# D-Hank/NeRF-tiny

Measured on AMD Instinct MI355X. Metric: rays/sec (64 coarse + 128 fine samples), lego 400x400, higher is better.
Workload: dtype f32

## Files before the change

### nerf-tiny_amd/csrc/field_bwd_reg.hip

```cpp
#include "field_common.h"

namespace nerf {

constexpr int RMB = 32;

template <int NFT>
struct WStageB {
  float4 w[NFT];
};

__device__ __forceinline__ float f4cb(const float4& v, int c) { return c == 0 ? v.x : (c == 1 ? v.y : (c == 2 ? v.z : v.w)); }

__device__ __forceinline__ unsigned mask_word(const uint16_t* __restrict__ mlayer, int t) { return mlayer[((t & 1) * 2) * 256 + (t >> 1) * 64]; }

template <int KB, int NFT, int NKB, int NNFT, bool ZERO_INIT, bool MASK_IN, bool STORE = true, bool HAS_NEXT_MASK = MASK_IN>
__device__ __forceinline__ void reg_layer_bwd(const int seg, const int next_seg , int lane,
                                              const f32x16* prev, f32x16* acc, WStageB<8>& st0, const uint16_t* __restrict__ mlayer,
                                              const uint16_t* __restrict__ mnext, unsigned& mfirst, float* __restrict__ grow, const RegBuf& rb) {
  constexpr int KT = KB / 4;
  WStageB<8> st1;
  const f32x16 zero = {0.f, 0.f, 0.f, 0.f, 0.f, 0.f, 0.f, 0.f, 0.f, 0.f, 0.f, 0.f, 0.f, 0.f, 0.f, 0.f};
  f32x16 tin[2];
  unsigned mw = mfirst;
  auto activate = [&](int t) {
    unsigned mn = 0;
    if (MASK_IN) {
      if (t + 1 < KT) mn = mask_word(mlayer, t + 1);
      else if (mnext != nullptr) mfirst = mask_word(mnext, 0);
    }
#pragma unroll
    for (int r = 0; r < 16; ++r) tin[t & 1][r] = MASK_IN ? (((mw >> r) & 1u) ? prev[t][r] : 0.f) : prev[t][r];
    if (grow == nullptr) {
#pragma unroll
      for (int r = 0; r < 16; ++r) asm volatile("" : "+v"(tin[t & 1][r]));
    }
    if (grow != nullptr) {
#pragma unroll
      for (int g = 0; g < 4; ++g)
        store_row4(grow + 32 * t + 8 * g, make_float4(tin[t & 1][4 * g], tin[t & 1][4 * g + 1], tin[t & 1][4 * g + 2], tin[t & 1][4 * g + 3]));
    }
    if (MASK_IN) mw = mn;
  };
  activate(0);
  auto kblock = [&](int kb, const WStageB<8>& cur, WStageB<8>& ld) {
    if (kb + 1 < KB) {
#pragma unroll
      for (int f = 0; f < NFT; ++f) ld.w[f] = reg_ldw(rb, seg + (int)(f * KB + kb + 1) * 64);
    } else if (next_seg >= 0) {
#pragma unroll
      for (int f = 0; f < NNFT; ++f) ld.w[f] = reg_ldw(rb, next_seg + (int)(f * NKB) * 64);
    }
    __builtin_amdgcn_sched_barrier(0);
    if ((kb & 3) == 2 && (kb >> 2) + 1 < KT) activate((kb >> 2) + 1);
#pragma unroll
    for (int s = 0; s < 4; ++s) {
      const float b = tin[(kb >> 2) & 1][4 * (kb & 3) + s];
#pragma unroll
      for (int f = 0; f < NFT; ++f) {
        if (ZERO_INIT && kb == 0 && s == 0)
          acc[f] = __builtin_amdgcn_mfma_f32_32x32x2f32(f4cb(cur.w[f], s), b, zero, 0, 0, 0);
        else
          acc[f] = __builtin_amdgcn_mfma_f32_32x32x2f32(f4cb(cur.w[f], s), b, acc[f], 0, 0, 0);
      }
    }
  };
#pragma unroll
  for (int kb = 0; kb < KB; kb += 2) {
    kblock(kb, st0, st1);
    kblock(kb + 1, st1, st0);
  }
}

template <int KB, int NKB, int NNFT, bool ZERO_INIT, bool STORE, bool HAS_NEXT_MASK>
__device__ __forceinline__ void reg_layer_bwd_thin(const int seg, const int next_seg , int lane,
                                                   const f32x16* prev, f32x16* acc, WStageB<8>& st0, const uint16_t* __restrict__ mlayer,
                                                   const uint16_t* __restrict__ mnext, unsigned& mfirst, float* __restrict__ grow, const RegBuf& rb) {
  static_assert(KB == 32, "ring indexing below assumes 32 k-blocks");
  constexpr int KT = KB / 4, D = 8;
  WStageB<8> st1;
  const f32x16 zero = {0.f, 0.f, 0.f, 0.f, 0.f, 0.f, 0.f, 0.f, 0.f, 0.f, 0.f, 0.f, 0.f, 0.f, 0.f, 0.f};
  f32x16 tin[2];
  unsigned mw = mfirst;
  auto slot = [&](int kb, int f) -> float4& { return ((kb % D) < 4) ? st0.w[2 * (kb % 4) + f] : st1.w[2 * (kb % 4) + f]; };
  auto activate = [&](int t) {
    unsigned mn = 0;
    if (t + 1 < KT) mn = mask_word(mlayer, t + 1);
    else if (HAS_NEXT_MASK) mfirst = mask_word(mnext, 0);
#pragma unroll
    for (int r = 0; r < 16; ++r) tin[t & 1][r] = ((mw >> r) & 1u) ? prev[t][r] : 0.f;
    if (STORE) {
#pragma unroll
      for (int g = 0; g < 4; ++g)
        store_row4(grow + 32 * t + 8 * g, make_float4(tin[t & 1][4 * g], tin[t & 1][4 * g + 1], tin[t & 1][4 * g + 2], tin[t & 1][4 * g + 3]));
    } else {
#pragma unroll
      for (int r = 0; r < 16; ++r) asm volatile("" : "+v"(tin[t & 1][r]));
    }
    mw = mn;
  };
#pragma unroll
  for (int kb = 1; kb < D; ++kb)
#pragma unroll
    for (int f = 0; f < 2; ++f) slot(kb, f) = reg_ldw(rb, seg + (int)(f * KB + kb) * 64);
  activate(0);
#pragma unroll
  for (int kb = 0; kb < KB; ++kb) {
    if ((kb & 3) == 2 && (kb >> 2) + 1 < KT) activate((kb >> 2) + 1);
    const float4 w0 = slot(kb, 0), w1 = slot(kb, 1);
#pragma unroll
    for (int s = 0; s < 4; ++s) {
      const float b = tin[(kb >> 2) & 1][4 * (kb & 3) + s];
      if (ZERO_INIT && kb == 0 && s == 0) {
        acc[0] = __builtin_amdgcn_mfma_f32_32x32x2f32(f4cb(w0, s), b, zero, 0, 0, 0);
        acc[1] = __builtin_amdgcn_mfma_f32_32x32x2f32(f4cb(w1, s), b, zero, 0, 0, 0);
      } else {
        acc[0] = __builtin_amdgcn_mfma_f32_32x32x2f32(f4cb(w0, s), b, acc[0], 0, 0, 0);
        acc[1] = __builtin_amdgcn_mfma_f32_32x32x2f32(f4cb(w1, s), b, acc[1], 0, 0, 0);
      }
    }
    __builtin_amdgcn_sched_barrier(0);
    if (kb + D < KB) {
#pragma unroll
      for (int f = 0; f < 2; ++f) slot(kb, f) = reg_ldw(rb, seg + (int)(f * KB + kb + D) * 64);
    } else if (kb == KB - 4 && next_seg >= 0) {
#pragma unroll
      for (int f = 0; f < NNFT; ++f) st0.w[f] = reg_ldw(rb, next_seg + (int)(f * NKB) * 64);
    }
    __builtin_amdgcn_sched_barrier(0);
  }
}

#ifdef NERF_STAMPS
#define BSTAMP(slot)                                            \
  do {                                                          \
    __builtin_amdgcn_sched_barrier(0);                          \
    const unsigned long long t_ = __builtin_readcyclecounter(); \
    __builtin_amdgcn_sched_barrier(0);                          \
    tsum[slot] += t_ - tlast;                                   \
    tlast = t_;                                                 \
  } while (0)
#else
#define BSTAMP(slot) do { } while (0)
#endif

template <bool FINE, bool QUERY = false, bool RGB = true>
__global__ __launch_bounds__(64, 1) void k_field_bwd_reg(const FieldBwdArgs a) {
  static_assert(FINE || !QUERY, "the query form carries the chain back to the points");
#ifdef NERF_STAMPS
  unsigned long long tsum[8] = {0, 0, 0, 0, 0, 0, 0, 0};
  unsigned long long tlast = __builtin_readcyclecounter();
#endif
  const int lane = threadIdx.x, j = lane & 31, h = lane >> 5;
  const int m0 = blockIdx.x * RMB;
  const int m = m0 + j;
  const bool valid = m < a.M;
  const int mc = valid ? m : a.M - 1;
  const size_t MS = (size_t)a.MSrows * WIDTH;
  const long long rrow = valid ? (long long)(a.row0 + m) : a.Mtot + j;
  const size_t grow_off = (size_t)rrow * WIDTH + 4 * h;
  float* const grow = a.G + grow_off;
  const float* const srow = a.save + grow_off;
  const uint16_t* const mrow = a.masks + ((size_t)(a.tile0 + (m0 >> 6)) * 4 + ((m0 >> 5) & 1)) * 256 + h * 32 + j;
  const size_t MKS = (size_t)a.tiles_tot * 4 * 256;
  const RegBuf rb = reg_buf(a.wp, threadIdx.x);
  constexpr int L256 = 8 * 32 * 64;
  const f32x16 zero = {0.f, 0.f, 0.f, 0.f, 0.f, 0.f, 0.f, 0.f, 0.f, 0.f, 0.f, 0.f, 0.f, 0.f, 0.f, 0.f};

  WStageB<8> st0;
  if constexpr (RGB) {
#pragma unroll
    for (int f = 0; f < 8; ++f) st0.w[f] = reg_ldw(rb, seg_off4(SEG_T_FOLD) + (f * 16) * 64);
  } else {
#pragma unroll
    for (int f = 0; f < 8; ++f) st0.w[f] = reg_ldw(rb, seg_off4(SEG_T_L7) + (f * 32) * 64);
  }
  auto mlayer = [&](int layer) { return mrow + (size_t)layer * MKS; };
  unsigned mfirst = mask_word(mlayer(7), 0);

  f32x16 D0[4];
  float ds;
  {
    const float* crow = QUERY ? a.save + (size_t)a.MSrows * QGRAD_GP + (size_t)rrow * QGRAD_C + 4 * h : srow + S_C * MS;
    float4 cv[4][4];
    float dz[3];
    if constexpr (RGB) {
#pragma unroll
      for (int t = 0; t < 4; ++t)
#pragma unroll
        for (int g = 0; g < 4; ++g) cv[t][g] = *reinterpret_cast<const float4*>(crow + 32 * t + 8 * g);
#pragma unroll
      for (int ch = 0; ch < 3; ++ch) {
        const float o = a.rgb[(size_t)mc * 3 + ch];
        const float up = a.drgb[(size_t)mc * 3 + ch];
        dz[ch] = valid ? up * ((1.0f - o) * o) : 0.f;
      }
    }
    const float sp = a.spre[a.row0 + mc];
    const float sgn = sp > 0.f ? 1.0f : (sp < 0.f ? -1.0f : 0.f);
    if constexpr (QUERY)
      ds = valid ? (a.dsig != nullptr ? a.dsig[mc] : 1.0f) * sgn : 0.f;
    else
      ds = valid ? a.dsig[mc] * sgn : 0.f;
    if (!QUERY && valid && h == 0) {
      *reinterpret_cast<float4*>(a.dz + (size_t)(a.row0 + m) * 4) = make_float4(dz[0], dz[1], dz[2], ds);
      a.dspre[a.row0 + m] = ds;
    }
    const float* wc = a.w.p[W_COLOR] + 4 * h;
#pragma unroll
    for (int t = 0; t < (RGB ? 4 : 0); ++t) {
      float4 q0[4], q1[4], q2[4];
#pragma unroll
      for (int g = 0; g < 4; ++g) {
        q0[g] = *reinterpret_cast<const float4*>(wc + 32 * t + 8 * g);
        q1[g] = *reinterpret_cast<const float4*>(wc + HALF + 32 * t + 8 * g);
        q2[g] = *reinterpret_cast<const float4*>(wc + 2 * HALF + 32 * t + 8 * g);
      }
      __builtin_amdgcn_sched_barrier(0);
#pragma unroll
      for (int g = 0; g < 4; ++g) {
        const float v0 = __builtin_fmaf(q2[g].x, dz[2], __builtin_fmaf(q1[g].x, dz[1], q0[g].x * dz[0]));
        const float v1 = __builtin_fmaf(q2[g].y, dz[2], __builtin_fmaf(q1[g].y, dz[1], q0[g].y * dz[0]));
        const float v2 = __builtin_fmaf(q2[g].z, dz[2], __builtin_fmaf(q1[g].z, dz[1], q0[g].z * dz[0]));
        const float v3 = __builtin_fmaf(q2[g].w, dz[2], __builtin_fmaf(q1[g].w, dz[1], q0[g].w * dz[0]));
        D0[t][4 * g + 0] = cv[t][g].x > 0.f ? v0 : 0.f;
        D0[t][4 * g + 1] = cv[t][g].y > 0.f ? v1 : 0.f;
        D0[t][4 * g + 2] = cv[t][g].z > 0.f ? v2 : 0.f;
        D0[t][4 * g + 3] = cv[t][g].w > 0.f ? v3 : 0.f;
      }
      __builtin_amdgcn_sched_barrier(0);
    }
  }
  BSTAMP(0);
  f32x16 A[8], B[8];
  {
    const float dsb = (h == 0) ? ds : 0.f;
    const float* ws = a.w.p[W_SIGMA];
#pragma unroll
    for (int f = 0; f < 8; ++f) B[f] = __builtin_amdgcn_mfma_f32_32x32x2f32(ws[f * 32 + j], dsb, zero, 0, 0, 0);
  }
  if constexpr (RGB)
    reg_layer_bwd<16, 8, 32, 8, false, false>(seg_off4(SEG_T_FOLD), seg_off4(SEG_T_L7), lane, D0, B, st0, nullptr, nullptr, mfirst,
                                              QUERY ? a.G : grow + G_D * MS, rb);
  BSTAMP(1);
  BSTAMP(2);
  constexpr int sT7 = seg_off4(SEG_T_L7);
  reg_layer_bwd<32, 8, 32, 8, true, true>(sT7, sT7 + L256, lane, B, A, st0, mlayer(7), mlayer(6), mfirst, QUERY ? a.G : grow + 7 * MS, rb);
  reg_layer_bwd<32, 8, 32, 8, true, true>(sT7 + L256, sT7 + 2 * L256, lane, A, B, st0, mlayer(6), mlayer(5), mfirst, QUERY ? a.G : grow + 6 * MS, rb);
  reg_layer_bwd<32, 8, 32, 8, true, true>(sT7 + 2 * L256, seg_off4(SEG_T_L4A), lane, B, A, st0, mlayer(5), mlayer(4), mfirst, QUERY ? a.G : grow + 5 * MS, rb);
  BSTAMP(3);
  f32x16 accg[2];
  if (FINE) {
    reg_layer_bwd<32, 8, 32, 2, true, true>(seg_off4(SEG_T_L4A), seg_off4(SEG_T_L4B), lane, A, B, st0, mlayer(4), mlayer(4), mfirst, QUERY ? a.G : grow + 4 * MS, rb);
    reg_layer_bwd_thin<32, 32, 8, true, false, true>(seg_off4(SEG_T_L4B), seg_off4(SEG_T_L3), lane, A, accg, st0, mlayer(4), mlayer(3), mfirst, nullptr, rb);
  } else {
    reg_layer_bwd<32, 8, 32, 8, true, true>(seg_off4(SEG_T_L4A), seg_off4(SEG_T_L3), lane, A, B, st0, mlayer(4), mlayer(3), mfirst, grow + 4 * MS, rb);
  }
  BSTAMP(4);
  constexpr int sT3 = seg_off4(SEG_T_L3);
  reg_layer_bwd<32, 8, 32, 8, true, true>(sT3, sT3 + L256, lane, B, A, st0, mlayer(3), mlayer(2), mfirst, QUERY ? a.G : grow + 3 * MS, rb);
  reg_layer_bwd<32, 8, 32, 8, true, true>(sT3 + L256, sT3 + 2 * L256, lane, A, B, st0, mlayer(2), mlayer(1), mfirst, QUERY ? a.G : grow + 2 * MS, rb);
  unsigned mb0[8];
  if (!FINE) {
#pragma unroll
    for (int t = 0; t < 8; ++t) mb0[t] = mask_word(mlayer(0), t);
  }
  reg_layer_bwd<32, 8, 32, 2, true, true, true, FINE>(sT3 + 2 * L256, FINE ? seg_off4(SEG_T_L0) : -1, lane, B, A, st0, mlayer(1),
                                                      mlayer(0), mfirst, QUERY ? a.G : grow + 1 * MS, rb);
  BSTAMP(5);
  if (FINE) {
    reg_layer_bwd_thin<32, 32, 2, false, !QUERY, false>(seg_off4(SEG_T_L0), -1, lane, A, accg, st0, mlayer(0), nullptr, mfirst,
                                                        QUERY ? nullptr : grow, rb);
    const int lane_e = __builtin_amdgcn_mbcnt_hi(~0u, __builtin_amdgcn_mbcnt_lo(~0u, 0u));
    const int j_e = lane_e & 31, h_e = lane_e >> 5;
    const int m_e = blockIdx.x * RMB + j_e;
    const bool valid_e = m_e < a.M;
    const int mc_e = valid_e ? m_e : a.M - 1;
    const long long rrow_e = valid_e ? (long long)(a.row0 + m_e) : a.Mtot + j_e;
    const float* rf = QUERY ? nullptr : a.rayf + (size_t)(mc_e / a.N) * RAYF;
    const float* gprow = QUERY ? a.save + (size_t)rrow_e * QGRAD_GP + 4 * h_e : a.save + (size_t)rrow_e * WIDTH + 4 * h_e + S_GP * ((size_t)a.MSrows * WIDTH);
    float4 gq[8];
#pragma unroll
    for (int g8 = 0; g8 < 8; ++g8) gq[g8] = *reinterpret_cast<const float4*>(gprow + 8 * g8);
    float dp[3] = {0.f, 0.f, 0.f};
#pragma unroll
    for (int g8 = 0; g8 < 8; ++g8)
#pragma unroll
      for (int e = 0; e < 2; ++e) {
        const int pi = 4 * g8 + 2 * h_e + e;
        if (pi < 30) {
          const int c = pi / 10, l = pi - 10 * c;
          const float fl = __uint_as_float(kFreqPointBits[l]);
          const float sn = e == 0 ? gq[g8].x : gq[g8].z, cn = e == 0 ? gq[g8].y : gq[g8].w;
          const float dgs = accg[g8 >> 2][4 * (g8 & 3) + 2 * e], dgc = accg[g8 >> 2][4 * (g8 & 3) + 2 * e + 1];
          const float contrib = fl * (cn * dgs - sn * dgc);
          if (c == 0) dp[0] += contrib; else if (c == 1) dp[1] += contrib; else dp[2] += contrib;
        }
      }
#pragma unroll
    for (int c = 0; c < 3; ++c) dp[c] += __shfl_xor(dp[c], 32);
    if (QUERY && valid_e && h_e == 0) {
#pragma unroll
      for (int c = 0; c < 3; ++c) a.dt[(size_t)m_e * 3 + c] = dp[c];
    }
    if (!QUERY && valid_e && h_e == 0) {
      const float dtp = __builtin_fmaf(rf[RF_DWRD + 2], dp[2], __builtin_fmaf(rf[RF_DWRD + 1], dp[1], rf[RF_DWRD] * dp[0]));
      a.dt[m_e] += dtp;
    }
  } else {
#pragma unroll
    for (int t = 0; t < 8; ++t)
#pragma unroll
      for (int g = 0; g < 4; ++g) {
        float4 v;
        v.x = ((mb0[t] >> (4 * g + 0)) & 1u) ? A[t][4 * g + 0] : 0.f;
        v.y = ((mb0[t] >> (4 * g + 1)) & 1u) ? A[t][4 * g + 1] : 0.f;
        v.z = ((mb0[t] >> (4 * g + 2)) & 1u) ? A[t][4 * g + 2] : 0.f;
        v.w = ((mb0[t] >> (4 * g + 3)) & 1u) ? A[t][4 * g + 3] : 0.f;
        store_row4(grow + 32 * t + 8 * g, v);
      }
  }
#ifdef NERF_STAMPS
  BSTAMP(6);
  if (a.stamps && lane == 0) {
    for (int i = 0; i < 7; ++i) atomicAdd(a.stamps + (FINE ? 8 : 0) + i, tsum[i]);
    atomicAdd(a.stamps + (FINE ? 30 : 31), 1ull);
  }
#endif
}

hipError_t launch_query_grad_bwd(const FieldBwdArgs& a, bool rgb, hipStream_t st) {
  if (a.M <= 0) return hipSuccess;
  const unsigned tiles = (unsigned)(((long long)a.M + RMB - 1) / RMB);
  if (rgb)
    hipLaunchKernelGGL((k_field_bwd_reg<true, true, true>), dim3(tiles), dim3(64), 0, st, a);
  else
    hipLaunchKernelGGL((k_field_bwd_reg<true, true, false>), dim3(tiles), dim3(64), 0, st, a);
  return hipGetLastError();
}

hipError_t launch_field_bwd_reg(const FieldBwdArgs& a, bool fine, hipStream_t st) {
  const int tiles = (a.M + RMB - 1) / RMB;
  if (fine)
    hipLaunchKernelGGL(k_field_bwd_reg<true>, dim3(tiles), dim3(64), 0, st, a);
  else
    hipLaunchKernelGGL(k_field_bwd_reg<false>, dim3(tiles), dim3(64), 0, st, a);
  return hipGetLastError();
}

}
```

### nerf-tiny_amd/csrc/field_fwd_reg.hip

```cpp
#include "field_common.h"
#include <type_traits>

namespace nerf {

constexpr int RM = 32;

template <int I0, int I1, class F>
__device__ __forceinline__ void static_for(F&& f) {
  if constexpr (I0 < I1) {
    f(std::integral_constant<int, I0>{});
    static_for<I0 + 1, I1>(f);
  }
}

template <int NFT>
struct WStage {
  float4 w[NFT];
};

template <int KB, int NFT>
__device__ __forceinline__ void stage_load(const float4* __restrict__ seg_lane, int kb, WStage<NFT>& s) {
#pragma unroll
  for (int f = 0; f < NFT; ++f) s.w[f] = seg_lane[(size_t)(f * KB + kb) * 64];
}

__device__ __forceinline__ float relu1(float x) { return __int_as_float(max(__float_as_int(x), 0)); }

__device__ __forceinline__ float f4c(const float4& v, int c) { return c == 0 ? v.x : (c == 1 ? v.y : (c == 2 ? v.z : v.w)); }

typedef int lds_i32 __attribute__((address_space(3), may_alias));
typedef int i32x4v __attribute__((ext_vector_type(4), may_alias));
typedef __attribute__((address_space(3))) i32x4v lds_i32x4;
constexpr int RELU_LDS_DWORDS = 2 * 4 * 64 * 4;
constexpr int COL_LDS_DWORDS = 3 * HALF + 4;
struct ReluLds {
  lds_i32* w;
  lds_i32* m[4];
};
__device__ __forceinline__ ReluLds relu_lds(lds_i32* base, int lane) {
  ReluLds L;
  L.w = base + 4 * lane;
#pragma unroll
  for (int c = 0; c < 4; ++c) L.m[c] = base + 4 * lane + ((c + (lane >> 3)) & 3);
  return L;
}
__device__ __forceinline__ float4 lds_ld4(const lds_i32* p) {
  const i32x4v v = *reinterpret_cast<const lds_i32x4*>(p);
  return make_float4(__int_as_float(v[0]), __int_as_float(v[1]), __int_as_float(v[2]), __int_as_float(v[3]));
}
template <typename DST>
__device__ __forceinline__ void relu_lds_op(const ReluLds& L, const f32x16& src, DST& dst, int dst0, int slot, int i) {
  const int g = i / 6, j = i - 6 * g, off = (slot * 4 + g) * 256;
  if (j == 0) {
    const i32x4v v = {__float_as_int(src[4 * g]), __float_as_int(src[4 * g + 1]), __float_as_int(src[4 * g + 2]), __float_as_int(src[4 * g + 3])};
    *reinterpret_cast<lds_i32x4*>(L.w + off) = v;
  } else if (j < 5) {
    __hip_atomic_fetch_max(L.m[j - 1] + off, 0, __ATOMIC_RELAXED, __HIP_MEMORY_SCOPE_WORKGROUP);
  } else {
    const i32x4v v = *reinterpret_cast<lds_i32x4*>(L.w + off);
#pragma unroll
    for (int c = 0; c < 4; ++c) dst[dst0 + c] = __int_as_float(v[c]);
  }
}

struct SaveIn {
  float* rows;
  uint16_t* mask;
};

__device__ __forceinline__ void bias_group(const float* b4h, int t, int g, f32x16& acc) {
  const float4 q = *reinterpret_cast<const float4*>(b4h + 32 * t + 8 * g);
  acc[4 * g + 0] = q.x;
  acc[4 * g + 1] = q.y;
  acc[4 * g + 2] = q.z;
  acc[4 * g + 3] = q.w;
}

template <int KB, int NFT, int NKB, int NNFT, bool ZERO_INIT, bool RELU_IN, int SAVE = 0, bool LDS_RELU = false, bool NEXT_RELU = false, int NEXT_BIAS = 0>
__device__ __forceinline__ void reg_layer(const int seg, const int next_seg , int lane,
                                          const f32x16* prev, f32x16* acc, WStage<8>& st0, const float* bv,
                                          const SaveIn sv, const RegBuf& rb, const ReluLds& rl, f32x4v& head,
                                          const float* nb = nullptr, f32x16* nacc = nullptr) {
  static_assert(!(LDS_RELU || NEXT_RELU || NEXT_BIAS) || SAVE != 1, "the saving forward keeps the VALU ReLU and the bias MFMAs");
  static_assert(NEXT_BIAS == 0 || ((LDS_RELU && RELU_IN) || NEXT_RELU), "the bias loads live in the stream with compile-time k-blocks");
  static_assert(NEXT_BIAS != 1 || (KB == 32 && RELU_IN), "NEXT_BIAS = 1 overwrites the 8 input tiles of a 256-wide ReLU layer");
  static_assert(NEXT_BIAS != 2 || KB == 8, "NEXT_BIAS = 2: one tile per k-block of layer 0");
  constexpr int KT = KB / 4;
  constexpr bool LR = LDS_RELU && RELU_IN;
  WStage<8> st1;
  const f32x16 zero = {0.f, 0.f, 0.f, 0.f, 0.f, 0.f, 0.f, 0.f, 0.f, 0.f, 0.f, 0.f, 0.f, 0.f, 0.f, 0.f};
  if (bv != nullptr) {
    const float one_h0 = (lane < 32) ? 1.0f : 0.0f;
#pragma unroll
    for (int f = 0; f < NFT; ++f) acc[f] = __builtin_amdgcn_mfma_f32_32x32x2f32(bv[f], one_h0, zero, 0, 0, 0);
  }
  f32x16 tin[2];
  if constexpr (LR) {
#pragma unroll
    for (int c = 0; c < 4; ++c) tin[0][c] = head[c];
    if (bv != nullptr) {
#pragma unroll
      for (int i = 6; i < 14; ++i) relu_lds_op(rl, prev[0], tin[0], 4 * (i / 6), 0, i);
#pragma unroll
      for (int i = 6; i < 14; ++i) {
        __builtin_amdgcn_sched_group_barrier(0x008, 1, 0);
        __builtin_amdgcn_sched_group_barrier(0x080, 1, 0);
      }
    }
  }
  [[maybe_unused]] const int lr0 = (bv != nullptr) ? 14 : 6;
  auto mask_word = [&](int t) {
    unsigned bits = 0;
#pragma unroll
    for (int r = 0; r < 16; ++r) bits |= (prev[t][r] > 0.f) ? (1u << r) : 0u;
    sv.mask[((t & 1) * 2) * 256 + (t >> 1) * 64] = (uint16_t)bits;
  };
  auto activate = [&](int t) {
    if constexpr (LR) {
      if (SAVE != 0) mask_word(t);
      return;
    }
#pragma unroll
    for (int r = 0; r < 16; ++r) tin[t & 1][r] = RELU_IN ? (SAVE == 1 ? fmaxf(prev[t][r], 0.f) : relu1(prev[t][r])) : prev[t][r];
#pragma unroll
    for (int r = 0; r < 16; ++r) asm volatile("" : "+v"(tin[t & 1][r]));
    if (SAVE == 1 || (SAVE == 2 && !RELU_IN)) {
#pragma unroll
      for (int g = 0; g < 4; ++g)
        store_row4(sv.rows + 32 * t + 8 * g, make_float4(tin[t & 1][4 * g], tin[t & 1][4 * g + 1], tin[t & 1][4 * g + 2], tin[t & 1][4 * g + 3]));
    }
    if (SAVE != 0 && RELU_IN) {
      unsigned bits = 0;
#pragma unroll
      for (int r = 0; r < 16; ++r) bits |= (prev[t][r] > 0.f) ? (1u << r) : 0u;
      sv.mask[((t & 1) * 2) * 256 + (t >> 1) * 64] = (uint16_t)bits;
    }
  };
  activate(0);
  if constexpr (!(LR || NEXT_RELU)) {
#pragma unroll
  for (int kb = 0; kb < KB; ++kb) {
    WStage<8>& ld = (kb & 1) ? st0 : st1;
    const WStage<8>& cur = (kb & 1) ? st1 : st0;
    if (kb + 1 < KB) {
#pragma unroll
      for (int f = 0; f < NFT; ++f) ld.w[f] = reg_ldw(rb, seg + (f * KB + kb + 1) * 64);
// ... 425 lines not shown
```

Before: 735,500.

## Use bfe-based mask selects and hoist epilogue loads ahead of MFMA layers

Replaces the shift/compare/select ReLU-mask logic with a single v_bfe_i32 sign-extend plus an AND per element, and narrows mask words to 16 bits. Hoists all colour-weight loads in the prologue out of the per-tile loop behind one scheduling barrier. In the fine path it issues the ray-direction and previous dt loads before the final thin MFMA layer so their latency overlaps compute, and rewrites the positional-encoding gradient reduction to be branch-free across the two half-waves. This costs extra live registers and replaces the read-modify-write of dt with a preloaded value.

New measurement: 735,800 (median of 2 runs). No clear change (+0.0%).

```diff
diff --git a/nerf-tiny_amd/csrc/field_bwd_reg.hip b/nerf-tiny_amd/csrc/field_bwd_reg.hip
--- a/nerf-tiny_amd/csrc/field_bwd_reg.hip
+++ b/nerf-tiny_amd/csrc/field_bwd_reg.hip
@@ -11,25 +11,31 @@
 
 __device__ __forceinline__ float f4cb(const float4& v, int c) { return c == 0 ? v.x : (c == 1 ? v.y : (c == 2 ? v.z : v.w)); }
 
-__device__ __forceinline__ unsigned mask_word(const uint16_t* __restrict__ mlayer, int t) { return mlayer[((t & 1) * 2) * 256 + (t >> 1) * 64]; }
+__device__ __forceinline__ uint16_t mask_word(const uint16_t* __restrict__ mlayer, int t) { return mlayer[((t & 1) * 2) * 256 + (t >> 1) * 64]; }
+
+__device__ __forceinline__ float mask_keep(float x, uint16_t mw, int r) {
+  int m;
+  asm("v_bfe_i32 %0, %1, %2, 1" : "=v"(m) : "v"(mw), "i"(r));
+  return __int_as_float(__float_as_int(x) & m);
+}
 
 template <int KB, int NFT, int NKB, int NNFT, bool ZERO_INIT, bool MASK_IN, bool STORE = true, bool HAS_NEXT_MASK = MASK_IN>
 __device__ __forceinline__ void reg_layer_bwd(const int seg, const int next_seg , int lane,
                                               const f32x16* prev, f32x16* acc, WStageB<8>& st0, const uint16_t* __restrict__ mlayer,
-                                              const uint16_t* __restrict__ mnext, unsigned& mfirst, float* __restrict__ grow, const RegBuf& rb) {
+                                              const uint16_t* __restrict__ mnext, uint16_t& mfirst, float* __restrict__ grow, const RegBuf& rb) {
   constexpr int KT = KB / 4;
   WStageB<8> st1;
   const f32x16 zero = {0.f, 0.f, 0.f, 0.f, 0.f, 0.f, 0.f, 0.f, 0.f, 0.f, 0.f, 0.f, 0.f, 0.f, 0.f, 0.f};
   f32x16 tin[2];
-  unsigned mw = mfirst;
+  uint16_t mw = mfirst;
   auto activate = [&](int t) {
-    unsigned mn = 0;
+    uint16_t mn = 0;
     if (MASK_IN) {
       if (t + 1 < KT) mn = mask_word(mlayer, t + 1);
       else if (mnext != nullptr) mfirst = mask_word(mnext, 0);
     }
 #pragma unroll
-    for (int r = 0; r < 16; ++r) tin[t & 1][r] = MASK_IN ? (((mw >> r) & 1u) ? prev[t][r] : 0.f) : prev[t][r];
+    for (int r = 0; r < 16; ++r) tin[t & 1][r] = MASK_IN ? mask_keep(prev[t][r], mw, r) : prev[t][r];
     if (grow == nullptr) {
 #pragma unroll
       for (int r = 0; r < 16; ++r) asm volatile("" : "+v"(tin[t & 1][r]));
@@ -74,20 +80,20 @@
 template <int KB, int NKB, int NNFT, bool ZERO_INIT, bool STORE, bool HAS_NEXT_MASK>
 __device__ __forceinline__ void reg_layer_bwd_thin(const int seg, const int next_seg , int lane,
                                                    const f32x16* prev, f32x16* acc, WStageB<8>& st0, const uint16_t* __restrict__ mlayer,
-                                                   const uint16_t* __restrict__ mnext, unsigned& mfirst, float* __restrict__ grow, const RegBuf& rb) {
+                                                   const uint16_t* __restrict__ mnext, uint16_t& mfirst, float* __restrict__ grow, const RegBuf& rb) {
   static_assert(KB == 32, "ring indexing below assumes 32 k-blocks");
   constexpr int KT = KB / 4, D = 8;
   WStageB<8> st1;
   const f32x16 zero = {0.f, 0.f, 0.f, 0.f, 0.f, 0.f, 0.f, 0.f, 0.f, 0.f, 0.f, 0.f, 0.f, 0.f, 0.f, 0.f};
   f32x16 tin[2];
-  unsigned mw = mfirst;
+  uint16_t mw = mfirst;
   auto slot = [&](int kb, int f) -> float4& { return ((kb % D) < 4) ? st0.w[2 * (kb % 4) + f] : st1.w[2 * (kb % 4) + f]; };
   auto activate = [&](int t) {
-    unsigned mn = 0;
+    uint16_t mn = 0;
     if (t + 1 < KT) mn = mask_word(mlayer, t + 1);
     else if (HAS_NEXT_MASK) mfirst = mask_word(mnext, 0);
 #pragma unroll
-    for (int r = 0; r < 16; ++r) tin[t & 1][r] = ((mw >> r) & 1u) ? prev[t][r] : 0.f;
+    for (int r = 0; r < 16; ++r) tin[t & 1][r] = mask_keep(prev[t][r], mw, r);
     if (STORE) {
 #pragma unroll
       for (int g = 0; g < 4; ++g)
@@ -175,60 +181,68 @@
     for (int f = 0; f < 8; ++f) st0.w[f] = reg_ldw(rb, seg_off4(SEG_T_L7) + (f * 32) * 64);
   }
   auto mlayer = [&](int layer) { return mrow + (size_t)layer * MKS; };
-  unsigned mfirst = mask_word(mlayer(7), 0);
+  uint16_t mfirst = mask_word(mlayer(7), 0);
 
   f32x16 D0[4];
   float ds;
   {
     const float* crow = QUERY ? a.save + (size_t)a.MSrows * QGRAD_GP + (size_t)rrow * QGRAD_C + 4 * h : srow + S_C * MS;
     float4 cv[4][4];
+    float o3[3] = {0.f, 0.f, 0.f}, up3[3] = {0.f, 0.f, 0.f};
+    if constexpr (RGB) {
+#pragma unroll
+      for (int t = 0; t < 4; ++t)
+#pragma unroll
+        for (int g = 0; g < 4; ++g) cv[t][g] = *reinterpret_cast<const float4*>(crow + 32 * t + 8 * g);
+#pragma unroll
+      for (int ch = 0; ch < 3; ++ch) {
+        o3[ch] = a.rgb[(size_t)mc * 3 + ch];
+        up3[ch] = a.drgb[(size_t)mc * 3 + ch];
+      }
+    }
+    const float sp = a.spre[a.row0 + mc];
+    float up_s;
+    if constexpr (QUERY)
+      up_s = a.dsig != nullptr ? a.dsig[mc] : 1.0f;
+    else
+      up_s = a.dsig[mc];
+    const float* wc = a.w.p[W_COLOR] + 4 * h;
+    float4 q0[RGB ? 4 : 1][4], q1[RGB ? 4 : 1][4], q2[RGB ? 4 : 1][4];
+#pragma unroll
+    for (int t = 0; t < (RGB ? 4 : 0); ++t)
+#pragma unroll
+      for (int g = 0; g < 4; ++g) {
+        q0[t][g] = *reinterpret_cast<const float4*>(wc + 32 * t + 8 * g);
+        q1[t][g] = *reinterpret_cast<const float4*>(wc + HALF + 32 * t + 8 * g);
+        q2[t][g] = *reinterpret_cast<const float4*>(wc + 2 * HALF + 32 * t + 8 * g);
+      }
+    __builtin_amdgcn_sched_barrier(0);
     float dz[3];
     if constexpr (RGB) {
 #pragma unroll
-      for (int t = 0; t < 4; ++t)
-#pragma unroll
-        for (int g = 0; g < 4; ++g) cv[t][g] = *reinterpret_cast<const float4*>(crow + 32 * t + 8 * g);
-#pragma unroll
-      for (int ch = 0; ch < 3; ++ch) {
-        const float o = a.rgb[(size_t)mc * 3 + ch];
-        const float up = a.drgb[(size_t)mc * 3 + ch];
-        dz[ch] = valid ? up * ((1.0f - o) * o) : 0.f;
-      }
-    }
-    const float sp = a.spre[a.row0 + mc];
+      for (int ch = 0; ch < 3; ++ch) dz[ch] = valid ? up3[ch] * ((1.0f - o3[ch]) * o3[ch]) : 0.f;
+    }
     const float sgn = sp > 0.f ? 1.0f : (sp < 0.f ? -1.0f : 0.f);
-    if constexpr (QUERY)
-      ds = valid ? (a.dsig != nullptr ? a.dsig[mc] : 1.0f) * sgn : 0.f;
-    else
-      ds = valid ? a.dsig[mc] * sgn : 0.f;
+    ds = valid ? up_s * sgn : 0.f;
     if (!QUERY && valid && h == 0) {
       *reinterpret_cast<float4*>(a.dz + (size_t)(a.row0 + m) * 4) = make_float4(dz[0], dz[1], dz[2], ds);
       a.dspre[a.row0 + m] = ds;
     }
-    const float* wc = a.w.p[W_COLOR] + 4 * h;
 #pragma unroll
     for (int t = 0; t < (RGB ? 4 : 0); ++t) {
-      float4 q0[4], q1[4], q2[4];
 #pragma unroll
       for (int g = 0; g < 4; ++g) {
-        q0[g] = *reinterpret_cast<const float4*>(wc + 32 * t + 8 * g);
-        q1[g] = *reinterpret_cast<const float4*>(wc + HALF + 32 * t + 8 * g);
-        q2[g] = *reinterpret_cast<const float4*>(wc + 2 * HALF + 32 * t + 8 * g);
-      }
-      __builtin_amdgcn_sched_barrier(0);
-#pragma unroll
-      for (int g = 0; g < 4; ++g) {
-        const float v0 = __builtin_fmaf(q2[g].x, dz[2], __builtin_fmaf(q1[g].x, dz[1], q0[g].x * dz[0]));
-        const float v1 = __builtin_fmaf(q2[g].y, dz[2], __builtin_fmaf(q1[g].y, dz[1], q0[g].y * dz[0]));
-        const float v2 = __builtin_fmaf(q2[g].z, dz[2], __builtin_fmaf(q1[g].z, dz[1], q0[g].z * dz[0]));
-        const float v3 = __builtin_fmaf(q2[g].w, dz[2], __builtin_fmaf(q1[g].w, dz[1], q0[g].w * dz[0]));
+        const float v0 = __builtin_fmaf(q2[t][g].x, dz[2], __builtin_fmaf(q1[t][g].x, dz[1], q0[t][g].x * dz[0]));
+        const float v1 = __builtin_fmaf(q2[t][g].y, dz[2], __builtin_fmaf(q1[t][g].y, dz[1], q0[t][g].y * dz[0]));
+        const float v2 = __builtin_fmaf(q2[t][g].z, dz[2], __builtin_fmaf(q1[t][g].z, dz[1], q0[t][g].z * dz[0]));
+        const float v3 = __builtin_fmaf(q2[t][g].w, dz[2], __builtin_fmaf(q1[t][g].w, dz[1], q0[t][g].w * dz[0]));
         D0[t][4 * g + 0] = cv[t][g].x > 0.f ? v0 : 0.f;
         D0[t][4 * g + 1] = cv[t][g].y > 0.f ? v1 : 0.f;
         D0[t][4 * g + 2] = cv[t][g].z > 0.f ? v2 : 0.f;
         D0[t][4 * g + 3] = cv[t][g].w > 0.f ? v3 : 0.f;
       }
-      __builtin_amdgcn_sched_barrier(0);
-    }
+    }
+    __builtin_amdgcn_sched_barrier(0);
   }
   BSTAMP(0);
   f32x16 A[8], B[8];
@@ -259,7 +273,7 @@
   constexpr int sT3 = seg_off4(SEG_T_L3);
   reg_layer_bwd<32, 8, 32, 8, true, true>(sT3, sT3 + L256, lane, B, A, st0, mlayer(3), mlayer(2), mfirst, QUERY ? a.G : grow + 3 * MS, rb);
   reg_layer_bwd<32, 8, 32, 8, true, true>(sT3 + L256, sT3 + 2 * L256, lane, A, B, st0, mlayer(2), mlayer(1), mfirst, QUERY ? a.G : grow + 2 * MS, rb);
-  unsigned mb0[8];
+  uint16_t mb0[8];
   if (!FINE) {
 #pragma unroll
     for (int t = 0; t < 8; ++t) mb0[t] = mask_word(mlayer(0), t);
@@ -268,8 +282,6 @@
                                                       mlayer(0), mfirst, QUERY ? a.G : grow + 1 * MS, rb);
   BSTAMP(5);
   if (FINE) {
-    reg_layer_bwd_thin<32, 32, 2, false, !QUERY, false>(seg_off4(SEG_T_L0), -1, lane, A, accg, st0, mlayer(0), nullptr, mfirst,
-                                                        QUERY ? nullptr : grow, rb);
     const int lane_e = __builtin_amdgcn_mbcnt_hi(~0u, __builtin_amdgcn_mbcnt_lo(~0u, 0u));
     const int j_e = lane_e & 31, h_e = lane_e >> 5;
     const int m_e = blockIdx.x * RMB + j_e;
@@ -281,19 +293,37 @@
     float4 gq[8];
 #pragma unroll
     for (int g8 = 0; g8 < 8; ++g8) gq[g8] = *reinterpret_cast<const float4*>(gprow + 8 * g8);
+    float dwrd[3] = {0.f, 0.f, 0.f}, dt_old = 0.f;
+    if (!QUERY) {
+#pragma unroll
+      for (int c = 0; c < 3; ++c) dwrd[c] = rf[RF_DWRD + c];
+      dt_old = a.dt[mc_e];
+    }
+    __builtin_amdgcn_sched_barrier(0);
+    reg_layer_bwd_thin<32, 32, 2, false, !QUERY, false>(seg_off4(SEG_T_L0), -1, lane, A, accg, st0, mlayer(0), nullptr, mfirst,
+                                                        QUERY ? nullptr : grow, rb);
+    const bool hi = h_e != 0;
     float dp[3] = {0.f, 0.f, 0.f};
 #pragma unroll
     for (int g8 = 0; g8 < 8; ++g8)
 #pragma unroll
       for (int e = 0; e < 2; ++e) {
-        const int pi = 4 * g8 + 2 * h_e + e;
-        if (pi < 30) {
-          const int c = pi / 10, l = pi - 10 * c;
-          const float fl = __uint_as_float(kFreqPointBits[l]);
-          const float sn = e == 0 ? gq[g8].x : gq[g8].z, cn = e == 0 ? gq[g8].y : gq[g8].w;
-          const float dgs = accg[g8 >> 2][4 * (g8 & 3) + 2 * e], dgc = accg[g8 >> 2][4 * (g8 & 3) + 2 * e + 1];
-          const float contrib = fl * (cn * dgs - sn * dgc);
-          if (c == 0) dp[0] += contrib; else if (c == 1) dp[1] += contrib; else dp[2] += contrib;
+        const int pa = 4 * g8 + e, pb = pa + 2;
+        const bool pad = pb >= 30;
+        const int ca = pa / 10, la = pa - 10 * ca, cb = pad ? ca : pb / 10, lb = pad ? la : pb - 10 * cb;
+        const float fa = __uint_as_float(kFreqPointLit[la]), fb = __uint_as_float(kFreqPointLit[lb]);
+        const float fl = (la == lb) ? fa : (hi ? fb : fa);
+        const float sn = e == 0 ? gq[g8].x : gq[g8].z, cn = e == 0 ? gq[g8].y : gq[g8].w;
+        const float dgs = accg[g8 >> 2][4 * (g8 & 3) + 2 * e], dgc = accg[g8 >> 2][4 * (g8 & 3) + 2 * e + 1];
+        const float contrib = fl * (cn * dgs - sn * dgc);
+        if (pad) {
+          dp[ca] = hi ? dp[ca] : dp[ca] + contrib;
+        } else if (ca == cb) {
+          dp[ca] += contrib;
+        } else {
+          const float sum = (hi ? dp[cb] : dp[ca]) + contrib;
+          dp[ca] = hi ? dp[ca] : sum;
+          dp[cb] = hi ? sum : dp[cb];
         }
       }
 #pragma unroll
@@ -303,21 +333,23 @@
       for (int c = 0; c < 3; ++c) a.dt[(size_t)m_e * 3 + c] = dp[c];
     }
     if (!QUERY && valid_e && h_e == 0) {
-      const float dtp = __builtin_fmaf(rf[RF_DWRD + 2], dp[2], __builtin_fmaf(rf[RF_DWRD + 1], dp[1], rf[RF_DWRD] * dp[0]));
-      a.dt[m_e] += dtp;
+      const float dtp = __builtin_fmaf(dwrd[2], dp[2], __builtin_fmaf(dwrd[1], dp[1], dwrd[0] * dp[0]));
+      a.dt[m_e] = dt_old + dtp;
     }
   } else {
 #pragma unroll
-    for (int t = 0; t < 8; ++t)
+    for (int t = 0; t < 8; ++t) {
+      const uint16_t mp = mb0[t];
 #pragma unroll
       for (int g = 0; g < 4; ++g) {
         float4 v;
-        v.x = ((mb0[t] >> (4 * g + 0)) & 1u) ? A[t][4 * g + 0] : 0.f;
-        v.y = ((mb0[t] >> (4 * g + 1)) & 1u) ? A[t][4 * g + 1] : 0.f;
-        v.z = ((mb0[t] >> (4 * g + 2)) & 1u) ? A[t][4 * g + 2] : 0.f;
-        v.w = ((mb0[t] >> (4 * g + 3)) & 1u) ? A[t][4 * g + 3] : 0.f;
+        v.x = mask_keep(A[t][4 * g + 0], mp, 4 * g + 0);
+        v.y = mask_keep(A[t][4 * g + 1], mp, 4 * g + 1);
+        v.z = mask_keep(A[t][4 * g + 2], mp, 4 * g + 2);
+        v.w = mask_keep(A[t][4 * g + 3], mp, 4 * g + 3);
         store_row4(grow + 32 * t + 8 * g, v);
       }
+    }
   }
 #ifdef NERF_STAMPS
   BSTAMP(6);
```

## Apply backward ReLU masks through LDS atomic-AND trips interleaved with MFMAs

Applied to the files above, without the earlier changes.

In the masked 256-wide backward layers, the per-element VALU mask selects are replaced by an LDS round trip: the next tile is written to LDS, masked with atomic AND against rotated sign-extended mask bits, and read back. These DS ops are interleaved one-for-one with MFMAs through sched_group_barrier, moving mask work off the VALU and overlapping it with matrix ops. The epilogue is also changed to prefetch gprow, ray-direction and dt loads before the last thin layer, and to unroll the frequency reduction at compile time with constant frequencies. This adds LDS usage and per-lane bit-rotation logic, and it depends on the lane-to-slot mapping matching the mask rotation exactly.

New measurement: 737,000 before, 733,600 after. Within noise of the previous version (-0.5%).

```diff
diff --git a/nerf-tiny_amd/csrc/field_bwd_reg.hip b/nerf-tiny_amd/csrc/field_bwd_reg.hip
--- a/nerf-tiny_amd/csrc/field_bwd_reg.hip
+++ b/nerf-tiny_amd/csrc/field_bwd_reg.hip
@@ -1,4 +1,5 @@
 #include "field_common.h"
+#include "lds_trip.h"
 
 namespace nerf {
 
@@ -13,35 +14,54 @@
 
 __device__ __forceinline__ unsigned mask_word(const uint16_t* __restrict__ mlayer, int t) { return mlayer[((t & 1) * 2) * 256 + (t >> 1) * 64]; }
 
+struct MaskRot {
+  unsigned k, k4, m;
+};
+__device__ __forceinline__ MaskRot mask_rot(int lane) {
+  MaskRot r;
+  r.k = (unsigned)(lane >> 3) & 3u;
+  r.k4 = 4u - r.k;
+  r.m = 0x1111u * ((1u << r.k4) - 1u);
+  return r;
+}
 template <int KB, int NFT, int NKB, int NNFT, bool ZERO_INIT, bool MASK_IN, bool STORE = true, bool HAS_NEXT_MASK = MASK_IN>
 __device__ __forceinline__ void reg_layer_bwd(const int seg, const int next_seg , int lane,
                                               const f32x16* prev, f32x16* acc, WStageB<8>& st0, const uint16_t* __restrict__ mlayer,
-                                              const uint16_t* __restrict__ mnext, unsigned& mfirst, float* __restrict__ grow, const RegBuf& rb) {
+                                              const uint16_t* __restrict__ mnext, unsigned& mfirst, float* __restrict__ grow, const RegBuf& rb,
+                                              const ReluLds& rl, const MaskRot& mr) {
+  static_assert(!MASK_IN || (KB == 32 && NFT == 8), "the DS schedule below is that of a 256-wide masked layer");
   constexpr int KT = KB / 4;
   WStageB<8> st1;
   const f32x16 zero = {0.f, 0.f, 0.f, 0.f, 0.f, 0.f, 0.f, 0.f, 0.f, 0.f, 0.f, 0.f, 0.f, 0.f, 0.f, 0.f};
   f32x16 tin[2];
   unsigned mw = mfirst;
-  auto activate = [&](int t) {
-    unsigned mn = 0;
+  unsigned mn = 0;
+  auto store_tile = [&](int t) {
+    if (grow != nullptr) {
+#pragma unroll
+      for (int g = 0; g < 4; ++g)
+        store_row4(grow + 32 * t + 8 * g, make_float4(tin[t & 1][4 * g], tin[t & 1][4 * g + 1], tin[t & 1][4 * g + 2], tin[t & 1][4 * g + 3]));
+    }
+  };
+  auto next_word = [&](int t) {
     if (MASK_IN) {
       if (t + 1 < KT) mn = mask_word(mlayer, t + 1);
       else if (mnext != nullptr) mfirst = mask_word(mnext, 0);
     }
+  };
+  auto activate = [&](int t) {
+    next_word(t);
 #pragma unroll
     for (int r = 0; r < 16; ++r) tin[t & 1][r] = MASK_IN ? (((mw >> r) & 1u) ? prev[t][r] : 0.f) : prev[t][r];
     if (grow == nullptr) {
 #pragma unroll
       for (int r = 0; r < 16; ++r) asm volatile("" : "+v"(tin[t & 1][r]));
     }
-    if (grow != nullptr) {
-#pragma unroll
-      for (int g = 0; g < 4; ++g)
-        store_row4(grow + 32 * t + 8 * g, make_float4(tin[t & 1][4 * g], tin[t & 1][4 * g + 1], tin[t & 1][4 * g + 2], tin[t & 1][4 * g + 3]));
-    }
+    store_tile(t);
     if (MASK_IN) mw = mn;
   };
   activate(0);
+  if constexpr (!MASK_IN) {
   auto kblock = [&](int kb, const WStageB<8>& cur, WStageB<8>& ld) {
     if (kb + 1 < KB) {
 #pragma unroll
@@ -68,6 +88,61 @@
   for (int kb = 0; kb < KB; kb += 2) {
     kblock(kb, st0, st1);
     kblock(kb + 1, st1, st0);
+  }
+  } else {
+  int mk[16];
+  static_for<0, KB>([&](auto kbc) __attribute__((always_inline)) {
+    constexpr int kb = decltype(kbc)::value, kt = kb >> 2, k4 = kb & 3;
+    constexpr bool trip = k4 == 2 && kt + 1 < KT;
+    WStageB<8>& ld = (kb & 1) ? st0 : st1;
+    const WStageB<8>& cur = (kb & 1) ? st1 : st0;
+    if (kb + 1 < KB) {
+#pragma unroll
+      for (int f = 0; f < NFT; ++f) ld.w[f] = reg_ldw(rb, seg + (int)(f * KB + kb + 1) * 64);
+    } else if (next_seg >= 0) {
+#pragma unroll
+      for (int f = 0; f < NNFT; ++f) ld.w[f] = reg_ldw(rb, next_seg + (int)(f * NKB) * 64);
+    }
+    __builtin_amdgcn_sched_barrier(0);
+    if constexpr (trip) {
+      next_word(kt + 1);
+      const unsigned rot = ((mw >> mr.k) & mr.m) | ((mw << mr.k4) & ~mr.m);
+#pragma unroll
+      for (int r = 0; r < 16; ++r) {
+        mk[r] = __builtin_amdgcn_sbfe((int)rot, r, 1);
+        asm volatile("" : "+v"(mk[r]));
+      }
+    }
+    if constexpr (k4 == 3 && kt + 1 < KT) {
+      store_tile(kt + 1);
+      mw = mn;
+    }
+#pragma unroll
+    for (int s = 0; s < 4; ++s) {
+      const float b = tin[kt & 1][4 * k4 + s];
+#pragma unroll
+      for (int f = 0; f < NFT; ++f) {
+        if (ZERO_INIT && kb == 0 && s == 0)
+          acc[f] = __builtin_amdgcn_mfma_f32_32x32x2f32(f4cb(cur.w[f], s), b, zero, 0, 0, 0);
+        else
+          acc[f] = __builtin_amdgcn_mfma_f32_32x32x2f32(f4cb(cur.w[f], s), b, acc[f], 0, 0, 0);
+        if constexpr (trip) {
+          const int i = 8 * s + f;
+          if (i < 24)
+            lds_trip_op(rl, prev[kt + 1], tin[(kt + 1) & 1], 4 * (i / 6), (kt + 1) & 1, i, [&](lds_i32* p, int g, int c) __attribute__((always_inline)) {
+              __hip_atomic_fetch_and(p, mk[4 * g + c], __ATOMIC_RELAXED, __HIP_MEMORY_SCOPE_WORKGROUP);
+            });
+        }
+      }
+    }
+    if constexpr (trip) {
+#pragma unroll
+      for (int i = 0; i < 32; ++i) {
+        __builtin_amdgcn_sched_group_barrier(0x008, 1, 0);
+        if (i < 24) __builtin_amdgcn_sched_group_barrier(0x080, 1, 0);
+      }
+    }
+  });
   }
 }
 
@@ -163,6 +238,9 @@
   const uint16_t* const mrow = a.masks + ((size_t)(a.tile0 + (m0 >> 6)) * 4 + ((m0 >> 5) & 1)) * 256 + h * 32 + j;
   const size_t MKS = (size_t)a.tiles_tot * 4 * 256;
   const RegBuf rb = reg_buf(a.wp, threadIdx.x);
+  __shared__ int mask_slots[RELU_LDS_DWORDS];
+  const ReluLds rl = relu_lds((lds_i32*)mask_slots, lane);
+  const MaskRot mr = mask_rot(lane);
   constexpr int L256 = 8 * 32 * 64;
   const f32x16 zero = {0.f, 0.f, 0.f, 0.f, 0.f, 0.f, 0.f, 0.f, 0.f, 0.f, 0.f, 0.f, 0.f, 0.f, 0.f, 0.f};
 
@@ -240,36 +318,34 @@
   }
   if constexpr (RGB)
     reg_layer_bwd<16, 8, 32, 8, false, false>(seg_off4(SEG_T_FOLD), seg_off4(SEG_T_L7), lane, D0, B, st0, nullptr, nullptr, mfirst,
-                                              QUERY ? a.G : grow + G_D * MS, rb);
+                                              QUERY ? a.G : grow + G_D * MS, rb, rl, mr);
   BSTAMP(1);
   BSTAMP(2);
   constexpr int sT7 = seg_off4(SEG_T_L7);
-  reg_layer_bwd<32, 8, 32, 8, true, true>(sT7, sT7 + L256, lane, B, A, st0, mlayer(7), mlayer(6), mfirst, QUERY ? a.G : grow + 7 * MS, rb);
-  reg_layer_bwd<32, 8, 32, 8, true, true>(sT7 + L256, sT7 + 2 * L256, lane, A, B, st0, mlayer(6), mlayer(5), mfirst, QUERY ? a.G : grow + 6 * MS, rb);
-  reg_layer_bwd<32, 8, 32, 8, true, true>(sT7 + 2 * L256, seg_off4(SEG_T_L4A), lane, B, A, st0, mlayer(5), mlayer(4), mfirst, QUERY ? a.G : grow + 5 * MS, rb);
+  reg_layer_bwd<32, 8, 32, 8, true, true>(sT7, sT7 + L256, lane, B, A, st0, mlayer(7), mlayer(6), mfirst, QUERY ? a.G : grow + 7 * MS, rb, rl, mr);
+  reg_layer_bwd<32, 8, 32, 8, true, true>(sT7 + L256, sT7 + 2 * L256, lane, A, B, st0, mlayer(6), mlayer(5), mfirst, QUERY ? a.G : grow + 6 * MS, rb, rl, mr);
+  reg_layer_bwd<32, 8, 32, 8, true, true>(sT7 + 2 * L256, seg_off4(SEG_T_L4A), lane, B, A, st0, mlayer(5), mlayer(4), mfirst, QUERY ? a.G : grow + 5 * MS, rb, rl, mr);
   BSTAMP(3);
   f32x16 accg[2];
   if (FINE) {
-    reg_layer_bwd<32, 8, 32, 2, true, true>(seg_off4(SEG_T_L4A), seg_off4(SEG_T_L4B), lane, A, B, st0, mlayer(4), mlayer(4), mfirst, QUERY ? a.G : grow + 4 * MS, rb);
+    reg_layer_bwd<32, 8, 32, 2, true, true>(seg_off4(SEG_T_L4A), seg_off4(SEG_T_L4B), lane, A, B, st0, mlayer(4), mlayer(4), mfirst, QUERY ? a.G : grow + 4 * MS, rb, rl, mr);
     reg_layer_bwd_thin<32, 32, 8, true, false, true>(seg_off4(SEG_T_L4B), seg_off4(SEG_T_L3), lane, A, accg, st0, mlayer(4), mlayer(3), mfirst, nullptr, rb);
   } else {
-    reg_layer_bwd<32, 8, 32, 8, true, true>(seg_off4(SEG_T_L4A), seg_off4(SEG_T_L3), lane, A, B, st0, mlayer(4), mlayer(3), mfirst, grow + 4 * MS, rb);
+    reg_layer_bwd<32, 8, 32, 8, true, true>(seg_off4(SEG_T_L4A), seg_off4(SEG_T_L3), lane, A, B, st0, mlayer(4), mlayer(3), mfirst, grow + 4 * MS, rb, rl, mr);
   }
   BSTAMP(4);
   constexpr int sT3 = seg_off4(SEG_T_L3);
-  reg_layer_bwd<32, 8, 32, 8, true, true>(sT3, sT3 + L256, lane, B, A, st0, mlayer(3), mlayer(2), mfirst, QUERY ? a.G : grow + 3 * MS, rb);
-  reg_layer_bwd<32, 8, 32, 8, true, true>(sT3 + L256, sT3 + 2 * L256, lane, A, B, st0, mlayer(2), mlayer(1), mfirst, QUERY ? a.G : grow + 2 * MS, rb);
+  reg_layer_bwd<32, 8, 32, 8, true, true>(sT3, sT3 + L256, lane, B, A, st0, mlayer(3), mlayer(2), mfirst, QUERY ? a.G : grow + 3 * MS, rb, rl, mr);
+  reg_layer_bwd<32, 8, 32, 8, true, true>(sT3 + L256, sT3 + 2 * L256, lane, A, B, st0, mlayer(2), mlayer(1), mfirst, QUERY ? a.G : grow + 2 * MS, rb, rl, mr);
   unsigned mb0[8];
   if (!FINE) {
 #pragma unroll
     for (int t = 0; t < 8; ++t) mb0[t] = mask_word(mlayer(0), t);
   }
   reg_layer_bwd<32, 8, 32, 2, true, true, true, FINE>(sT3 + 2 * L256, FINE ? seg_off4(SEG_T_L0) : -1, lane, B, A, st0, mlayer(1),
-                                                      mlayer(0), mfirst, QUERY ? a.G : grow + 1 * MS, rb);
+                                                      mlayer(0), mfirst, QUERY ? a.G : grow + 1 * MS, rb, rl, mr);
   BSTAMP(5);
   if (FINE) {
-    reg_layer_bwd_thin<32, 32, 2, false, !QUERY, false>(seg_off4(SEG_T_L0), -1, lane, A, accg, st0, mlayer(0), nullptr, mfirst,
-                                                        QUERY ? nullptr : grow, rb);
     const int lane_e = __builtin_amdgcn_mbcnt_hi(~0u, __builtin_amdgcn_mbcnt_lo(~0u, 0u));
     const int j_e = lane_e & 31, h_e = lane_e >> 5;
     const int m_e = blockIdx.x * RMB + j_e;
@@ -279,23 +355,42 @@
     const float* rf = QUERY ? nullptr : a.rayf + (size_t)(mc_e / a.N) * RAYF;
     const float* gprow = QUERY ? a.save + (size_t)rrow_e * QGRAD_GP + 4 * h_e : a.save + (size_t)rrow_e * WIDTH + 4 * h_e + S_GP * ((size_t)a.MSrows * WIDTH);
     float4 gq[8];
-#pragma unroll
-    for (int g8 = 0; g8 < 8; ++g8) gq[g8] = *reinterpret_cast<const float4*>(gprow + 8 * g8);
+    float rfd[3] = {0.f, 0.f, 0.f}, dt0 = 0.f;
+    auto epilogue_loads = [&]() {
+#pragma unroll
+      for (int g8 = 0; g8 < 8; ++g8) gq[g8] = *reinterpret_cast<const float4*>(gprow + 8 * g8);
+      if constexpr (!QUERY) {
+#pragma unroll
+        for (int c = 0; c < 3; ++c) rfd[c] = rf[RF_DWRD + c];
+        dt0 = a.dt[mc_e];
+      }
+      __builtin_amdgcn_sched_barrier(0);
+    };
+    if constexpr (!QUERY) epilogue_loads();
+    reg_layer_bwd_thin<32, 32, 2, false, !QUERY, false>(seg_off4(SEG_T_L0), -1, lane, A, accg, st0, mlayer(0), nullptr, mfirst,
+                                                        QUERY ? nullptr : grow, rb);
+    if constexpr (QUERY) epilogue_loads();
     float dp[3] = {0.f, 0.f, 0.f};
-#pragma unroll
-    for (int g8 = 0; g8 < 8; ++g8)
-#pragma unroll
-      for (int e = 0; e < 2; ++e) {
-        const int pi = 4 * g8 + 2 * h_e + e;
-        if (pi < 30) {
-          const int c = pi / 10, l = pi - 10 * c;
-          const float fl = __uint_as_float(kFreqPointBits[l]);
-          const float sn = e == 0 ? gq[g8].x : gq[g8].z, cn = e == 0 ? gq[g8].y : gq[g8].w;
-          const float dgs = accg[g8 >> 2][4 * (g8 & 3) + 2 * e], dgc = accg[g8 >> 2][4 * (g8 & 3) + 2 * e + 1];
-          const float contrib = fl * (cn * dgs - sn * dgc);
-          if (c == 0) dp[0] += contrib; else if (c == 1) dp[1] += contrib; else dp[2] += contrib;
-        }
-      }
+    static_for<0, 16>([&](auto ic) __attribute__((always_inline)) {
+      constexpr int g8 = decltype(ic)::value >> 1, e = decltype(ic)::value & 1;
+      constexpr int pa = 4 * g8 + e, pb = pa + 2;
+      constexpr bool pad = pb >= 30;
+      constexpr int ca = pa / 10, la = pa - 10 * ca, cb = pad ? ca : pb / 10, lb = pad ? la : pb - 10 * cb;
+      static_assert(pa < 30, "lane half 0 never pads");
+      constexpr uint32_t fa = kFreqPointLit[la], fb = kFreqPointLit[lb];
+      const float fl = (la == lb) ? __uint_as_float(fa) : (h_e ? __uint_as_float(fb) : __uint_as_float(fa));
+      const float sn = e == 0 ? gq[g8].x : gq[g8].z, cn = e == 0 ? gq[g8].y : gq[g8].w;
+      const float dgs = accg[g8 >> 2][4 * (g8 & 3) + 2 * e], dgc = accg[g8 >> 2][4 * (g8 & 3) + 2 * e + 1];
+      const float contrib = fl * (cn * dgs - sn * dgc);
+      if constexpr (pad) {
+        dp[ca] += h_e ? 0.f : contrib;
+      } else if constexpr (ca == cb) {
+        dp[ca] += contrib;
+      } else {
+        dp[ca] += h_e ? 0.f : contrib;
+        dp[cb] += h_e ? contrib : 0.f;
+      }
+    });
 #pragma unroll
     for (int c = 0; c < 3; ++c) dp[c] += __shfl_xor(dp[c], 32);
     if (QUERY && valid_e && h_e == 0) {
@@ -303,8 +398,8 @@
       for (int c = 0; c < 3; ++c) a.dt[(size_t)m_e * 3 + c] = dp[c];
     }
     if (!QUERY && valid_e && h_e == 0) {
-      const float dtp = __builtin_fmaf(rf[RF_DWRD + 2], dp[2], __builtin_fmaf(rf[RF_DWRD + 1], dp[1], rf[RF_DWRD] * dp[0]));
-      a.dt[m_e] += dtp;
+      const float dtp = __builtin_fmaf(rfd[2], dp[2], __builtin_fmaf(rfd[1], dp[1], rfd[0] * dp[0]));
+      a.dt[m_e] = dt0 + dtp;
     }
   } else {
 #pragma unroll
diff --git a/nerf-tiny_amd/csrc/field_fwd_reg.hip b/nerf-tiny_amd/csrc/field_fwd_reg.hip
--- a/nerf-tiny_amd/csrc/field_fwd_reg.hip
+++ b/nerf-tiny_amd/csrc/field_fwd_reg.hip
@@ -1,17 +1,10 @@
 #include "field_common.h"
+#include "lds_trip.h"
 #include <type_traits>
 
 namespace nerf {
 
 constexpr int RM = 32;
-
-template <int I0, int I1, class F>
-__device__ __forceinline__ void static_for(F&& f) {
-  if constexpr (I0 < I1) {
-    f(std::integral_constant<int, I0>{});
-    static_for<I0 + 1, I1>(f);
-  }
-}
 
 template <int NFT>
 struct WStage {
@@ -28,40 +21,7 @@
 
 __device__ __forceinline__ float f4c(const float4& v, int c) { return c == 0 ? v.x : (c == 1 ? v.y : (c == 2 ? v.z : v.w)); }
 
-typedef int lds_i32 __attribute__((address_space(3), may_alias));
-typedef int i32x4v __attribute__((ext_vector_type(4), may_alias));
-typedef __attribute__((address_space(3))) i32x4v lds_i32x4;
-constexpr int RELU_LDS_DWORDS = 2 * 4 * 64 * 4;
 constexpr int COL_LDS_DWORDS = 3 * HALF + 4;
-struct ReluLds {
-  lds_i32* w;
-  lds_i32* m[4];
-};
-__device__ __forceinline__ ReluLds relu_lds(lds_i32* base, int lane) {
-  ReluLds L;
-  L.w = base + 4 * lane;
-#pragma unroll
-  for (int c = 0; c < 4; ++c) L.m[c] = base + 4 * lane + ((c + (lane >> 3)) & 3);
-  return L;
-}
-__device__ __forceinline__ float4 lds_ld4(const lds_i32* p) {
-  const i32x4v v = *reinterpret_cast<const lds_i32x4*>(p);
-  return make_float4(__int_as_float(v[0]), __int_as_float(v[1]), __int_as_float(v[2]), __int_as_float(v[3]));
-}
-template <typename DST>
-__device__ __forceinline__ void relu_lds_op(const ReluLds& L, const f32x16& src, DST& dst, int dst0, int slot, int i) {
-  const int g = i / 6, j = i - 6 * g, off = (slot * 4 + g) * 256;
-  if (j == 0) {
-    const i32x4v v = {__float_as_int(src[4 * g]), __float_as_int(src[4 * g + 1]), __float_as_int(src[4 * g + 2]), __float_as_int(src[4 * g + 3])};
-    *reinterpret_cast<lds_i32x4*>(L.w + off) = v;
-  } else if (j < 5) {
-    __hip_atomic_fetch_max(L.m[j - 1] + off, 0, __ATOMIC_RELAXED, __HIP_MEMORY_SCOPE_WORKGROUP);
-  } else {
-    const i32x4v v = *reinterpret_cast<lds_i32x4*>(L.w + off);
-#pragma unroll
-    for (int c = 0; c < 4; ++c) dst[dst0 + c] = __int_as_float(v[c]);
-  }
-}
 
 struct SaveIn {
   float* rows;
diff --git a/nerf-tiny_amd/csrc/lds_trip.h b/nerf-tiny_amd/csrc/lds_trip.h
--- /dev/null
+++ b/nerf-tiny_amd/csrc/lds_trip.h
@@ -0,0 +1,53 @@
+#pragma once
+#include "field_common.h"
+#include <type_traits>
+
+namespace nerf {
+
+template <int I0, int I1, class F>
+__device__ __forceinline__ void static_for(F&& f) {
+  if constexpr (I0 < I1) {
+    f(std::integral_constant<int, I0>{});
+    static_for<I0 + 1, I1>(f);
+  }
+}
+
+typedef int lds_i32 __attribute__((address_space(3), may_alias));
+typedef int i32x4v __attribute__((ext_vector_type(4), may_alias));
+typedef __attribute__((address_space(3))) i32x4v lds_i32x4;
+constexpr int RELU_LDS_DWORDS = 2 * 4 * 64 * 4;
+struct ReluLds {
+  lds_i32* w;
+  lds_i32* m[4];
+};
+__device__ __forceinline__ ReluLds relu_lds(lds_i32* base, int lane) {
+  ReluLds L;
+  L.w = base + 4 * lane;
+#pragma unroll
+  for (int c = 0; c < 4; ++c) L.m[c] = base + 4 * lane + ((c + (lane >> 3)) & 3);
+  return L;
+}
+__device__ __forceinline__ float4 lds_ld4(const lds_i32* p) {
+  const i32x4v v = *reinterpret_cast<const lds_i32x4*>(p);
+  return make_float4(__int_as_float(v[0]), __int_as_float(v[1]), __int_as_float(v[2]), __int_as_float(v[3]));
+}
+template <typename DST, typename OP>
+__device__ __forceinline__ void lds_trip_op(const ReluLds& L, const f32x16& src, DST& dst, int dst0, int slot, int i, OP&& op) {
+  const int g = i / 6, j = i - 6 * g, off = (slot * 4 + g) * 256;
+  if (j == 0) {
+    const i32x4v v = {__float_as_int(src[4 * g]), __float_as_int(src[4 * g + 1]), __float_as_int(src[4 * g + 2]), __float_as_int(src[4 * g + 3])};
+    *reinterpret_cast<lds_i32x4*>(L.w + off) = v;
+  } else if (j < 5) {
+    op(L.m[j - 1] + off, g, j - 1);
+  } else {
+    const i32x4v v = *reinterpret_cast<lds_i32x4*>(L.w + off);
+#pragma unroll
+    for (int c = 0; c < 4; ++c) dst[dst0 + c] = __int_as_float(v[c]);
+  }
+}
+template <typename DST>
+__device__ __forceinline__ void relu_lds_op(const ReluLds& L, const f32x16& src, DST& dst, int dst0, int slot, int i) {
+  lds_trip_op(L, src, dst, dst0, slot, i, [](lds_i32* p, int, int) __attribute__((always_inline)) { __hip_atomic_fetch_max(p, 0, __ATOMIC_RELAXED, __HIP_MEMORY_SCOPE_WORKGROUP); });
+}
+
+}
```
